# renegade-fi/mpc-jellyfish

Measured on AMD Instinct MI355X. Metric: msm_g1_scalar_pairs_per_s, higher is better.
Workload: dtype u32 (381-bit Fq as 14 x 29-bit limbs, Montgomery)

## Files before the change

mpc-jellyfish_amd/csrc/ecx.cuh:

```cuda
#pragma once
#include "ec.cuh"
#include "fx.cuh"

namespace mzk {

template <class X>
struct AffineX {
    Fx<X> x, y;
    MZK_HD bool is_inf() const {
        uint32_t a = 0;
#pragma unroll
        for (int i = 0; i < X::XN; i++) a |= x.l[i] | y.l[i];
        return a == 0;
    }
};

template <class X>
struct XYZZX {
    Fx<X> x, y, zz, zzz;
    MZK_HD bool is_inf() const {
        uint32_t a = 0;
#pragma unroll
        for (int i = 0; i < X::XN; i++) a |= zz.l[i];
        return a == 0;
    }
    MZK_HD static XYZZX inf() {
        XYZZX r;
        r.x = Fx<X>::one(); r.y = Fx<X>::one(); r.zz = Fx<X>::zero(); r.zzz = Fx<X>::zero();
        return r;
    }
    MZK_HD static XYZZX from_affine(const AffineX<X>& p) {
        if (p.is_inf()) return inf();
        XYZZX r;
        r.x = p.x; r.y = p.y; r.zz = Fx<X>::one(); r.zzz = Fx<X>::one();
        return r;
    }
};

template <class X>
MZK_HD Fx<X> fx_neg_m(const Fx<X>& y) {
    Fx<X> r;
#pragma unroll
    for (int i = 0; i < X::XN; i++) r.l[i] = X::XSUB2[i] - y.l[i];
    return r;
}

template <class X>
MZK_HD XYZZX<X> xyzzx_dbl_affine(const AffineX<X>& p) {
    XYZZX<X> r;
    const Fx<X> u = fx_norm(fx_add(p.y, p.y));
    const Fx<X> v = fx_sqr(u);
    const Fx<X> w = fx_mul(u, v);
    const Fx<X> s = fx_mul(p.x, v);
    const Fx<X> x2 = fx_sqr(p.x);
    const Fx<X> m = fx_norm(fx_add(fx_add(x2, x2), x2));
    const Fx<X> mm = fx_sqr(m);
    r.x = fx_norm(fx_sub_pad<X>(mm, fx_add(s, s), X::XSUB_2S));
    const Fx<X> d = fx_norm(fx_sub_pad<X>(s, r.x, X::XSUB_XY));
    r.y = fx_norm(fx_sub2(fx_mul(m, d), fx_mul(w, p.y)));
    r.zz = v;
    r.zzz = w;
    return r;
}

template <class X>
MZK_HD XYZZX<X> xyzzx_dbl(const XYZZX<X>& p) {
    if (p.is_inf()) return p;
    XYZZX<X> r;
    const Fx<X> u = fx_norm(fx_add(p.y, p.y));
    const Fx<X> v = fx_sqr(u);
    const Fx<X> w = fx_mul(u, v);
    const Fx<X> s = fx_mul(p.x, v);
    const Fx<X> x2 = fx_sqr(p.x);
    const Fx<X> m = fx_norm(fx_add(fx_add(x2, x2), x2));
    const Fx<X> mm = fx_sqr(m);
    r.x = fx_norm(fx_sub_pad<X>(mm, fx_add(s, s), X::XSUB_2S));
    const Fx<X> d = fx_norm(fx_sub_pad<X>(s, r.x, X::XSUB_XY));
    r.y = fx_norm(fx_sub2(fx_mul(m, d), fx_mul(w, p.y)));
    r.zz = fx_mul(v, p.zz);
    r.zzz = fx_mul(w, p.zzz);
    return r;
}

template <class X>
MZK_HD XYZZX<X> xyzzx_madd(const XYZZX<X>& p, const AffineX<X>& q, bool negate) {
    if (q.is_inf()) return p;
    const Fx<X> qy = negate ? fx_neg_m(q.y) : q.y;
    if (p.is_inf()) {
        XYZZX<X> r;
        r.x = q.x; r.y = fx_norm(qy); r.zz = Fx<X>::one(); r.zzz = Fx<X>::one();
        return r;
    }
    const Fx<X> u2 = fx_mul(q.x, p.zz);
    const Fx<X> s2 = fx_mul(qy, p.zzz);
    const Fx<X> pp_ = fx_norm(fx_sub_pad<X>(u2, p.x, X::XSUB_XY));
    const Fx<X> rr_ = fx_norm(fx_sub_pad<X>(s2, p.y, X::XSUB_XY));
    const Fx<X> pp = fx_sqr(pp_);
    const Fx<X> rr2 = fx_sqr(rr_);
    if (fx_is_zero_m(pp)) {
        if (fx_is_zero_m(rr2)) {
            AffineX<X> qq;
            qq.x = q.x;
            qq.y = fx_norm(qy);
            return xyzzx_dbl_affine(qq);
        }
        return XYZZX<X>::inf();
    }
    XYZZX<X> r;
    const Fx<X> ppp = fx_mul(pp_, pp);
    const Fx<X> qv = fx_mul(p.x, pp);
    r.x = fx_norm(fx_sub_pad<X>(rr2, fx_add(ppp, fx_add(qv, qv)), X::XSUB_PQ));
    const Fx<X> d = fx_norm(fx_sub_pad<X>(qv, r.x, X::XSUB_XY));
    r.y = fx_mul2(rr_, d, p.y, fx_neg_m(ppp));
    r.zz = fx_mul(p.zz, pp);
    r.zzz = fx_mul(p.zzz, ppp);
    return r;
}

template <class X>
MZK_HD XYZZX<X> xyzzx_add(const XYZZX<X>& p, const XYZZX<X>& q) {
    if (q.is_inf()) return p;
    if (p.is_inf()) return q;
    const Fx<X> u1 = fx_mul(p.x, q.zz), u2 = fx_mul(q.x, p.zz);
    const Fx<X> s1 = fx_mul(p.y, q.zzz), s2 = fx_mul(q.y, p.zzz);
    const Fx<X> pp_ = fx_norm(fx_sub2(u2, u1));
    const Fx<X> rr_ = fx_norm(fx_sub2(s2, s1));
    const Fx<X> pp = fx_sqr(pp_);
    const Fx<X> rr2 = fx_sqr(rr_);
    if (fx_is_zero_m(pp)) {
        if (fx_is_zero_m(rr2)) return xyzzx_dbl(p);
        return XYZZX<X>::inf();
    }
    XYZZX<X> r;
    const Fx<X> ppp = fx_mul(pp_, pp);
    const Fx<X> qv = fx_mul(u1, pp);
    r.x = fx_norm(fx_sub_pad<X>(rr2, fx_add(ppp, fx_add(qv, qv)), X::XSUB_PQ));
    const Fx<X> d = fx_norm(fx_sub_pad<X>(qv, r.x, X::XSUB_XY));
    r.y = fx_mul2(rr_, d, s1, fx_neg_m(ppp));
    r.zz = fx_mul(fx_mul(p.zz, q.zz), pp);
    r.zzz = fx_mul(fx_mul(p.zzz, q.zzz), ppp);
    return r;
}

#if defined(__HIPCC__)
template <int CTRL, class X>
__device__ __forceinline__ Fx<X> fx_quad_perm(const Fx<X>& a) {
    Fx<X> r;
#pragma unroll
    for (int i = 0; i < X::XN; i++) r.l[i] = (uint32_t)__builtin_amdgcn_update_dpp(0, (int)a.l[i], CTRL, 0xF, 0xF, true);
    return r;
}
template <class X>
__device__ __forceinline__ Fx<X> fx_sel(bool c, const Fx<X>& a, const Fx<X>& b) {
    Fx<X> r;
#pragma unroll
    for (int i = 0; i < X::XN; i++) r.l[i] = c ? a.l[i] : b.l[i];
    return r;
}
constexpr int QP_SWAP2 = 0x4E, QP_SWAP1 = 0xB1, QP_L0 = 0x00, QP_L1 = 0x55, QP_L2 = 0xAA, QP_L3 = 0xFF;

template <class X>
__device__ __forceinline__ Fx<X> xyzzx_add_quad(const Fx<X>& ca, const Fx<X>& cb, int role) {
    const bool r0 = role == 0, r1 = role == 1, hi = role >= 2;
    uint32_t za = 0, zb = 0;
#pragma unroll
    for (int i = 0; i < X::XN; i++) { za |= ca.l[i]; zb |= cb.l[i]; }
    int special = (role == 2 && (za == 0 || zb == 0)) ? 1 : 0;
    const Fx<X> p1 = fx_mul(ca, fx_quad_perm<QP_SWAP2>(cb));
    const Fx<X> d = fx_norm(fx_sub2(fx_quad_perm<QP_SWAP2>(p1), p1));
    const Fx<X> p2 = fx_mul(fx_sel(hi, ca, d), fx_sel(hi, cb, d));
    if (r0 && fx_is_zero_m(p2)) special = 1;
    special |= __builtin_amdgcn_update_dpp(0, special, QP_SWAP1, 0xF, 0xF, true);
    special |= __builtin_amdgcn_update_dpp(0, special, QP_SWAP2, 0xF, 0xF, true);
    if (special) {
        XYZZX<X> a, b;
        a.x = fx_quad_perm<QP_L0>(ca); a.y = fx_quad_perm<QP_L1>(ca); a.zz = fx_quad_perm<QP_L2>(ca); a.zzz = fx_quad_perm<QP_L3>(ca);
        b.x = fx_quad_perm<QP_L0>(cb); b.y = fx_quad_perm<QP_L1>(cb); b.zz = fx_quad_perm<QP_L2>(cb); b.zzz = fx_quad_perm<QP_L3>(cb);
        const XYZZX<X> r = xyzzx_add(a, b);
        return fx_sel(hi, fx_sel(role == 2, r.zz, r.zzz), fx_sel(r0, r.x, r.y));
    }
    const Fx<X> pp = fx_quad_perm<QP_L0>(p2);
    const Fx<X> u1 = fx_quad_perm<QP_L0>(p1);
    const Fx<X> p3 = fx_mul(fx_sel(r0, d, fx_sel(r1, u1, p2)), pp);
    const Fx<X> ppp = fx_quad_perm<QP_L0>(p3);
    const Fx<X> x3 = fx_norm(fx_sub_pad<X>(p2, fx_add(ppp, fx_add(p3, p3)), X::XSUB_PQ));
    const Fx<X> qx = fx_norm(fx_sub_pad<X>(p3, x3, X::XSUB_XY));
    const Fx<X> s1 = fx_quad_perm<QP_L1>(p1);
    const Fx<X> p4 = fx_mul(fx_sel(r0, s1, fx_sel(r1, d, p2)), fx_sel(r1, qx, ppp));
    const Fx<X> y3 = fx_norm(fx_sub2(p4, fx_quad_perm<QP_L0>(p4)));
    const Fx<X> x3_0 = fx_quad_perm<QP_L1>(x3);
    return fx_sel(hi, fx_sel(role == 2, p3, p4), fx_sel(r0, x3_0, y3));
}
#endif

template <class X>
MZK_HD XYZZ<Fp<X>> xyzzx_to_boundary(const XYZZX<X>& p) {
    XYZZ<Fp<X>> r;
    if (p.is_inf()) return XYZZ<Fp<X>>::inf();
    r.x = fx_to_boundary<X>(p.x); r.y = fx_to_boundary<X>(p.y);
    r.zz = fx_to_boundary<X>(p.zz); r.zzz = fx_to_boundary<X>(p.zzz);
    return r;
}

}
```

mpc-jellyfish_amd/csrc/ecz.cuh:

```cuda
#pragma once
#include "ecx.cuh"
#include "fz.cuh"

namespace mzk {

template <class Z>
struct AffineZ {
    Fz<Z> x, y;
    MZK_HD bool is_inf() const {
        int32_t a = 0;
#pragma unroll
        for (int i = 0; i < Z::ZN; i++) a |= x.l[i] | y.l[i];
        return a == 0;
    }
};

template <class Z>
struct XYZZZ {
    Fz<Z> x, y, zz, zzz;
    MZK_HD bool is_inf() const { return fz_is_zero(zz); }
    MZK_HD static XYZZZ inf() {
        XYZZZ r;
        r.x = Fz<Z>::one(); r.y = Fz<Z>::one(); r.zz = Fz<Z>::zero(); r.zzz = Fz<Z>::zero();
        return r;
    }
    MZK_HD static XYZZZ from_affine(const AffineZ<Z>& p) {
        if (p.is_inf()) return inf();
        XYZZZ r;
        r.x = p.x; r.y = p.y; r.zz = Fz<Z>::one(); r.zzz = Fz<Z>::one();
        return r;
    }
};

template <class Z>
MZK_HD void ecz_xy3(Fz<Z>& x3, Fz<Z>& y3, const Fz<Z>& a, const Fz<Z>& b_plus_2c, const Fz<Z>& q, const Fz<Z>& r, const Fz<Z>& y, const Fz<Z>& ppp) {
    x3 = fz_norm_wide(fz_sub(a, b_plus_2c));
    const Fz<Z> d = fz_norm(fz_sub(q, x3));
    y3 = fz_mul2(r, d, y, fz_neg(ppp));
}

template <class Z>
MZK_HD XYZZZ<Z> xyzzz_dbl_affine(const AffineZ<Z>& p) {
    XYZZZ<Z> r;
    const Fz<Z> u = fz_norm(fz_add(p.y, p.y));
    const Fz<Z> v = fz_sqr(u);
    const Fz<Z> w = fz_mul(u, v);
    const Fz<Z> s = fz_mul(p.x, v);
    const Fz<Z> x2 = fz_sqr(p.x);
    const Fz<Z> m = fz_norm_wide(fz_add(fz_add(x2, x2), x2));
    const Fz<Z> mm = fz_sqr(m);
    ecz_xy3<Z>(r.x, r.y, mm, fz_add(s, s), s, m, p.y, w);
    r.zz = v;
    r.zzz = w;
    return r;
}

template <class Z>
MZK_HD XYZZZ<Z> xyzzz_dbl(const XYZZZ<Z>& p) {
    if (p.is_inf()) return p;
    XYZZZ<Z> r;
    const Fz<Z> u = fz_norm(fz_add(p.y, p.y));
    const Fz<Z> v = fz_sqr(u);
    const Fz<Z> w = fz_mul(u, v);
    const Fz<Z> s = fz_mul(p.x, v);
    const Fz<Z> x2 = fz_sqr(p.x);
    const Fz<Z> m = fz_norm_wide(fz_add(fz_add(x2, x2), x2));
    const Fz<Z> mm = fz_sqr(m);
    ecz_xy3<Z>(r.x, r.y, mm, fz_add(s, s), s, m, p.y, w);
    r.zz = fz_mul(v, p.zz);
    r.zzz = fz_mul(w, p.zzz);
    return r;
}

template <class Z>
MZK_HD XYZZZ<Z> xyzzz_madd(const XYZZZ<Z>& p, const AffineZ<Z>& q, bool negate) {
    if (q.is_inf()) return p;
    const Fz<Z> qy = negate ? fz_neg(q.y) : q.y;
    if (p.is_inf()) {
        XYZZZ<Z> r;
        r.x = q.x; r.y = qy; r.zz = Fz<Z>::one(); r.zzz = Fz<Z>::one();
        return r;
    }
    const Fz<Z> u2 = fz_mul(q.x, p.zz);
    const Fz<Z> s2 = fz_mul(qy, p.zzz);
    const Fz<Z> pp_ = fz_norm(fz_sub(u2, p.x));
    const Fz<Z> rr_ = fz_norm(fz_sub(s2, p.y));
    const Fz<Z> pp = fz_sqr(pp_);
    const Fz<Z> rr2 = fz_sqr(rr_);
    if (fz_is_zero(pp)) {
        if (fz_is_zero(rr2)) {
            AffineZ<Z> qq;
            qq.x = q.x;
            qq.y = qy;
            return xyzzz_dbl_affine(qq);
        }
        return XYZZZ<Z>::inf();
    }
    XYZZZ<Z> r;
    const Fz<Z> ppp = fz_mul(pp_, pp);
    const Fz<Z> qv = fz_mul(p.x, pp);
    ecz_xy3<Z>(r.x, r.y, rr2, fz_add(ppp, fz_add(qv, qv)), qv, rr_, p.y, ppp);
    r.zz = fz_mul(p.zz, pp);
    r.zzz = fz_mul(p.zzz, ppp);
    return r;
}

template <class Z>
MZK_HD XYZZZ<Z> xyzzz_add(const XYZZZ<Z>& p, const XYZZZ<Z>& q) {
    if (q.is_inf()) return p;
    if (p.is_inf()) return q;
    const Fz<Z> u1 = fz_mul(p.x, q.zz), u2 = fz_mul(q.x, p.zz);
    const Fz<Z> s1 = fz_mul(p.y, q.zzz), s2 = fz_mul(q.y, p.zzz);
    const Fz<Z> pp_ = fz_norm(fz_sub(u2, u1));
    const Fz<Z> rr_ = fz_norm(fz_sub(s2, s1));
    const Fz<Z> pp = fz_sqr(pp_);
    const Fz<Z> rr2 = fz_sqr(rr_);
    if (fz_is_zero(pp)) {
        if (fz_is_zero(rr2)) return xyzzz_dbl(p);
        return XYZZZ<Z>::inf();
    }
    XYZZZ<Z> r;
    const Fz<Z> ppp = fz_mul(pp_, pp);
    const Fz<Z> qv = fz_mul(u1, pp);
    ecz_xy3<Z>(r.x, r.y, rr2, fz_add(ppp, fz_add(qv, qv)), qv, rr_, s1, ppp);
    r.zz = fz_mul(fz_mul(p.zz, q.zz), pp);
    r.zzz = fz_mul(fz_mul(p.zzz, q.zzz), ppp);
    return r;
}

#if defined(__HIPCC__)
template <int CTRL, class Z>
__device__ __forceinline__ Fz<Z> fz_quad_perm(const Fz<Z>& a) {
    Fz<Z> r;
#pragma unroll
    for (int i = 0; i < Z::ZN; i++) {
        r.l[i] = __builtin_amdgcn_update_dpp(0, a.l[i], CTRL, 0xF, 0xF, true);
        asm("" : "+v"(r.l[i]));
    }
    return r;
}
template <class Z>
__device__ __forceinline__ Fz<Z> fz_sel(bool c, const Fz<Z>& a, const Fz<Z>& b) {
    Fz<Z> r;
#pragma unroll
    for (int i = 0; i < Z::ZN; i++) r.l[i] = c ? a.l[i] : b.l[i];
    return r;
}

template <class Z>
__device__ __forceinline__ Fz<Z> xyzzz_add_quad(const Fz<Z>& ca, const Fz<Z>& cb, int role) {
    const bool r0 = role == 0, r1 = role == 1, hi = role >= 2;
    int special = (role == 2 && (fz_is_zero(ca) || fz_is_zero(cb))) ? 1 : 0;
    const Fz<Z> p1 = fz_mul(ca, fz_quad_perm<QP_SWAP2>(cb));
    const Fz<Z> d = fz_norm(fz_sub(fz_quad_perm<QP_SWAP2>(p1), p1));
    const Fz<Z> p2 = fz_mul(fz_sel(hi, ca, d), fz_sel(hi, cb, d));
    if (r0 && fz_is_zero(p2)) special = 1;
    special |= __builtin_amdgcn_update_dpp(0, special, QP_SWAP1, 0xF, 0xF, true);
    special |= __builtin_amdgcn_update_dpp(0, special, QP_SWAP2, 0xF, 0xF, true);
    if (special) {
        XYZZZ<Z> a, b;
        a.x = fz_quad_perm<QP_L0>(ca); a.y = fz_quad_perm<QP_L1>(ca); a.zz = fz_quad_perm<QP_L2>(ca); a.zzz = fz_quad_perm<QP_L3>(ca);
        b.x = fz_quad_perm<QP_L0>(cb); b.y = fz_quad_perm<QP_L1>(cb); b.zz = fz_quad_perm<QP_L2>(cb); b.zzz = fz_quad_perm<QP_L3>(cb);
        const XYZZZ<Z> r = xyzzz_add(a, b);
        return fz_sel(hi, fz_sel(role == 2, r.zz, r.zzz), fz_sel(r0, r.x, r.y));
    }
    const Fz<Z> pp = fz_quad_perm<QP_L0>(p2);
    const Fz<Z> u1 = fz_quad_perm<QP_L0>(p1);
    const Fz<Z> p3 = fz_mul(fz_sel(r0, d, fz_sel(r1, u1, p2)), pp);
    const Fz<Z> ppp = fz_quad_perm<QP_L0>(p3);
    const Fz<Z> x3 = fz_norm_wide(fz_sub(p2, fz_add(ppp, fz_add(p3, p3))));
    const Fz<Z> qx = fz_norm(fz_sub(p3, x3));
    const Fz<Z> s1 = fz_quad_perm<QP_L1>(p1);
    const Fz<Z> p4 = fz_mul(fz_sel(r0, s1, fz_sel(r1, d, p2)), fz_sel(r1, qx, ppp));
    const Fz<Z> y3 = fz_norm(fz_sub(p4, fz_quad_perm<QP_L0>(p4)));
    const Fz<Z> x3_0 = fz_quad_perm<QP_L1>(x3);
    return fz_sel(hi, fz_sel(role == 2, p3, p4), fz_sel(r0, x3_0, y3));
}
#endif

template <class Z>
MZK_HD XYZZ<Fp<Z>> xyzzz_to_boundary(const XYZZZ<Z>& p) {
    XYZZ<Fp<Z>> r;
    if (p.is_inf()) return XYZZ<Fp<Z>>::inf();
    r.x = fz_to_boundary<Z>(p.x); r.y = fz_to_boundary<Z>(p.y);
    r.zz = fz_to_boundary<Z>(p.zz); r.zzz = fz_to_boundary<Z>(p.zzz);
    return r;
}

}
```

mpc-jellyfish_amd/csrc/msm.cuh:

```cuda
#pragma once
#include <hip/hip_runtime.h>

#include "ec.cuh"
#include "ecx.cuh"
#include "ecz.cuh"

namespace mzk {

constexpr int MSM_THREADS = 256;
constexpr int MSM_ACC_THREADS = 128;
constexpr uint32_t MSM_HEAVY_PER_THREAD = 16;
constexpr uint32_t MSM_HEAVY_RUN = MSM_ACC_THREADS * MSM_HEAVY_PER_THREAD;
constexpr uint32_t MSM_HEAVY_FANIN = MSM_ACC_THREADS * 32;
constexpr int MSM_HEAVY_COUNTERS = 6;
__host__ __device__ inline bool msm_is_heavy(uint32_t count, uint32_t cap) { return count > cap + MSM_HEAVY_RUN; }

inline int msm_choose_window(unsigned long long n) {
    int lg = 0;
    while ((1ull << (lg + 1)) <= n) lg++;
    int c = lg - 2;
    if (c < 4) c = 4;
    if (c > 16) c = 16;
    return c;
}
// ... 86 lines not shown
__global__ __launch_bounds__(1024) void msm_scan_kernel(const uint32_t* __restrict__ hist, uint32_t* __restrict__ offs, uint32_t M) {
    __shared__ uint32_t part[1024];
    const int w = blockIdx.x, t = threadIdx.x;
    const uint32_t per = (M + 1023) / 1024;
    const uint32_t lo = t * per, hi = min(M, lo + per);
    uint32_t sum = 0;
    for (uint32_t b = lo; b < hi; b++) sum += hist[(size_t)w * M + b];
    part[t] = sum;
    __syncthreads();
    for (int d = 1; d < 1024; d <<= 1) {
        uint32_t v = t >= d ? part[t - d] : 0;
        __syncthreads();
        part[t] += v;
        __syncthreads();
    }
    uint32_t run = part[t] - sum;
    for (uint32_t b = lo; b < hi; b++) {
        offs[(size_t)w * M + b] = run;
        run += hist[(size_t)w * M + b];
    }
}

constexpr uint32_t MSM_ORDER_SLICE = 8192;
__device__ __forceinline__ uint32_t order_key(uint32_t count) { return 1023u - min(count, 1023u); }

__global__ __launch_bounds__(1024) void msm_order_hist_kernel(const uint32_t* __restrict__ hist, uint32_t M, uint32_t* __restrict__ keycnt) {
    __shared__ uint32_t cnt[1024];
    const uint32_t w = blockIdx.y, t = threadIdx.x;
    const uint32_t lo = blockIdx.x * MSM_ORDER_SLICE, hi = min(M, lo + MSM_ORDER_SLICE);
    cnt[t] = 0;
    __syncthreads();
    for (uint32_t b = lo + t; b < hi; b += 1024) atomicAdd(&cnt[order_key(hist[(size_t)w * M + b])], 1u);
    __syncthreads();
    if (cnt[t]) atomicAdd(&keycnt[(size_t)w * 1024 + t], cnt[t]);
}
__global__ __launch_bounds__(1024) void msm_order_scan_kernel(uint32_t* __restrict__ keycnt, uint32_t global_sets) {
    __shared__ uint32_t part[1024];
    const uint32_t w = blockIdx.x, t = threadIdx.x;
    uint32_t mine = keycnt[(size_t)w * 1024 + t];
    for (uint32_t s = 1; s < global_sets; s++) mine += keycnt[(size_t)s * 1024 + t];
    part[t] = mine;
    __syncthreads();
    for (int d = 1; d < 1024; d <<= 1) {
        uint32_t v = t >= (uint32_t)d ? part[t - d] : 0;
        __syncthreads();
        part[t] += v;
        __syncthreads();
    }
    keycnt[(size_t)w * 1024 + t] = part[t] - mine;
}
__global__ __launch_bounds__(1024) void msm_order_scatter_kernel(const uint32_t* __restrict__ hist, uint32_t M, uint32_t* __restrict__ keycur,
                                                                 uint32_t* __restrict__ order, bool global) {
    __shared__ uint32_t cnt[1024];
    const uint32_t w = blockIdx.y, t = threadIdx.x;
    const uint32_t row = global ? 0u : w;
    const uint32_t lo = blockIdx.x * MSM_ORDER_SLICE, hi = min(M, lo + MSM_ORDER_SLICE);
    cnt[t] = 0;
    __syncthreads();
    for (uint32_t b = lo + t; b < hi; b += 1024) atomicAdd(&cnt[order_key(hist[(size_t)w * M + b])], 1u);
    __syncthreads();
    const uint32_t mine = cnt[t];
    __syncthreads();
    cnt[t] = mine ? atomicAdd(&keycur[(size_t)row * 1024 + t], mine) : 0u;
    __syncthreads();
    for (uint32_t b = lo + t; b < hi; b += 1024) {
        const uint32_t pos = atomicAdd(&cnt[order_key(hist[(size_t)w * M + b])], 1u);
        order[(size_t)row * M + pos] = w * M + b;
    }
}

struct LongDesc;
struct HeavyRun;
__device__ __forceinline__ void msm_long_register(uint32_t w, uint32_t b, uint32_t c, uint32_t offs_t, int n_win, uint32_t cap, uint32_t desc_cap,
                                                  LongDesc* __restrict__ desc, uint32_t* __restrict__ desc_count, uint32_t run_cap,
                                                  uint32_t h1_cap, HeavyRun* __restrict__ heavy_runs);
__global__ __launch_bounds__(1024) void msm_order_place_kernel(const uint32_t* __restrict__ hist, const uint32_t* __restrict__ offs, uint32_t M,
                                                               const uint32_t* __restrict__ keycnt, uint32_t* __restrict__ keycur, uint32_t* __restrict__ order,
                                                               int n_win, uint32_t cap, uint32_t desc_cap, LongDesc* __restrict__ desc,
                                                               uint32_t* __restrict__ desc_count, uint32_t run_cap, uint32_t h1_cap, HeavyRun* __restrict__ heavy_runs,
                                                               bool global) {
    __shared__ uint32_t cnt[1024];
    __shared__ uint32_t part[1024];
    const uint32_t w = blockIdx.y, t = threadIdx.x;
    const uint32_t row = global ? 0u : w;
    const uint32_t lo = blockIdx.x * MSM_ORDER_SLICE, hi = min(M, lo + MSM_ORDER_SLICE);
    uint32_t total = 0;
    if (global) for (uint32_t s = 0; s < gridDim.y; s++) total += keycnt[(size_t)s * 1024 + t];
    else total = keycnt[(size_t)w * 1024 + t];
    part[t] = total;
    cnt[t] = 0;
    __syncthreads();
    for (int d = 1; d < 1024; d <<= 1) {
        uint32_t v = t >= (uint32_t)d ? part[t - d] : 0;
        __syncthreads();
        part[t] += v;
        __syncthreads();
    }
    const uint32_t key_start = part[t] - total;
    for (uint32_t b = lo + t; b < hi; b += 1024) atomicAdd(&cnt[order_key(hist[(size_t)w * M + b])], 1u);
    __syncthreads();
    const uint32_t mine = cnt[t];
    __syncthreads();
    cnt[t] = mine ? key_start + atomicAdd(&keycur[(size_t)row * 1024 + t], mine) : 0u;
    __syncthreads();
    for (uint32_t b = lo + t; b < hi; b += 1024) {
        const uint32_t c = hist[(size_t)w * M + b];
        const uint32_t pos = atomicAdd(&cnt[order_key(c)], 1u);
        order[(size_t)row * M + pos] = w * M + b;
        if (desc_count && c > cap) msm_long_register(w, b, c, offs[(size_t)w * M + b], n_win, cap, desc_cap, desc, desc_count, run_cap, h1_cap, heavy_runs);
    }
}

template <class FQ>
__device__ __forceinline__ Affine<Fp<FQ>> load_affine(const uint32_t* __restrict__ bases, unsigned long long idx) {
    Affine<Fp<FQ>> p;
    const uint32_t* src = bases + idx * (2 * FQ::N);
    p.x = load_fp<FQ>(src);
    p.y = load_fp<FQ>(src + FQ::N);
    return p;
}
template <class FQ>
__device__ __forceinline__ XYZZ<Fp<FQ>> load_xyzz(const uint32_t* __restrict__ buf, unsigned long long idx) {
    XYZZ<Fp<FQ>> p;
    const uint32_t* src = buf + idx * (4 * FQ::N);
    p.x = load_fp<FQ>(src);
    p.y = load_fp<FQ>(src + FQ::N);
    p.zz = load_fp<FQ>(src + 2 * FQ::N);
    p.zzz = load_fp<FQ>(src + 3 * FQ::N);
    return p;
}
template <class FQ>
__device__ __forceinline__ void store_xyzz(uint32_t* __restrict__ buf, unsigned long long idx, const XYZZ<Fp<FQ>>& p) {
    uint32_t* dst = buf + idx * (4 * FQ::N);
    store_fp<FQ>(dst, p.x);
    store_fp<FQ>(dst + FQ::N, p.y);
    store_fp<FQ>(dst + 2 * FQ::N, p.zz);
    store_fp<FQ>(dst + 3 * FQ::N, p.zzz);
}

template <class FQ>
struct EcFp {
    using Field = FQ;
    using Aff = Affine<Fp<FQ>>;
    using Pt = XYZZ<Fp<FQ>>;
    static constexpr int AFF_WORDS = 2 * FQ::N, PT_WORDS = 4 * FQ::N;
    static __device__ __forceinline__ Aff load_aff(const uint32_t* __restrict__ bases, unsigned long long idx) { return load_affine<FQ>(bases, idx); }
    static __device__ __forceinline__ Pt load_pt(const uint32_t* __restrict__ buf, unsigned long long idx) { return load_xyzz<FQ>(buf, idx); }
    static __device__ __forceinline__ void store_pt(uint32_t* __restrict__ buf, unsigned long long idx, const Pt& p) { store_xyzz<FQ>(buf, idx, p); }
    static __device__ __forceinline__ Pt inf() { return Pt::inf(); }
    static __device__ __forceinline__ Pt madd(const Pt& a, Aff q, bool negate) {
        if (negate) q.y = neg(q.y);
        return xyzz_madd(a, q);
    }
    static __device__ __forceinline__ Pt add(const Pt& a, const Pt& b) { return xyzz_add(a, b); }
    static __device__ __forceinline__ XYZZ<Fp<FQ>> to_boundary(const Pt& p) { return p; }
};

template <class X>
__device__ __forceinline__ void load_words(uint32_t* dst, const uint32_t* __restrict__ src, int n_words) {
    for (int i = 0; i < n_words / 4; i++) {
        const uint4 v = reinterpret_cast<const uint4*>(src)[i];
        dst[4 * i] = v.x; dst[4 * i + 1] = v.y; dst[4 * i + 2] = v.z; dst[4 * i + 3] = v.w;
    }
}

template <class X>
struct EcFx {
    using Field = X;
    using Aff = AffineX<X>;
    using Pt = XYZZX<X>;
    using Fe = Fx<X>;
    static constexpr int LIMBS = X::XN, SLOT_WORDS = X::XN;
    static constexpr int AFF_WORDS = 2 * X::XN, PT_WORDS = 4 * X::XN;
    static_assert((4 * X::XN) % 4 == 0 && (2 * X::XN) % 2 == 0, "points are whole 16-byte / 8-byte words");
    static __device__ __forceinline__ Aff load_aff(const uint32_t* __restrict__ bases, unsigned long long idx) {
        uint32_t w[AFF_WORDS];
        if constexpr (AFF_WORDS % 4 == 0) {
            const uint4* src = reinterpret_cast<const uint4*>(bases + idx * AFF_WORDS);
#pragma unroll
            for (int i = 0; i < AFF_WORDS / 4; i++) {
                const uint4 v = src[i];
                w[4 * i] = v.x; w[4 * i + 1] = v.y; w[4 * i + 2] = v.z; w[4 * i + 3] = v.w;
            }
        } else {
            const uint2* src = reinterpret_cast<const uint2*>(bases + idx * AFF_WORDS);
#pragma unroll
            for (int i = 0; i < AFF_WORDS / 2; i++) {
                const uint2 v = src[i];
                w[2 * i] = v.x; w[2 * i + 1] = v.y;
            }
        }
        Aff p;
#pragma unroll
        for (int i = 0; i < X::XN; i++) { p.x.l[i] = w[i]; p.y.l[i] = w[X::XN + i]; }
        return p;
    }
    static __device__ __forceinline__ Pt load_pt(const uint32_t* __restrict__ buf, unsigned long long idx) {
        uint32_t w[PT_WORDS];
        const uint4* src = reinterpret_cast<const uint4*>(buf + idx * PT_WORDS);
#pragma unroll
        for (int i = 0; i < PT_WORDS / 4; i++) {
            const uint4 v = src[i];
            w[4 * i] = v.x; w[4 * i + 1] = v.y; w[4 * i + 2] = v.z; w[4 * i + 3] = v.w;
        }
        Pt p;
#pragma unroll
        for (int i = 0; i < X::XN; i++) {
            p.x.l[i] = w[i]; p.y.l[i] = w[X::XN + i]; p.zz.l[i] = w[2 * X::XN + i]; p.zzz.l[i] = w[3 * X::XN + i];
        }
        return p;
    }
    static __device__ __forceinline__ void store_pt(uint32_t* __restrict__ buf, unsigned long long idx, const Pt& p) {
        uint32_t w[PT_WORDS];
#pragma unroll
        for (int i = 0; i < X::XN; i++) {
            w[i] = p.x.l[i]; w[X::XN + i] = p.y.l[i]; w[2 * X::XN + i] = p.zz.l[i]; w[3 * X::XN + i] = p.zzz.l[i];
        }
        uint4* dst = reinterpret_cast<uint4*>(buf + idx * PT_WORDS);
#pragma unroll
        for (int i = 0; i < PT_WORDS / 4; i++) dst[i] = make_uint4(w[4 * i], w[4 * i + 1], w[4 * i + 2], w[4 * i + 3]);
    }
    static __device__ __forceinline__ Pt inf() { return Pt::inf(); }
    static __device__ __forceinline__ Pt madd(const Pt& a, const Aff& q, bool negate) { return xyzzx_madd(a, q, negate); }
    static __device__ __forceinline__ Pt add(const Pt& a, const Pt& b) { return xyzzx_add(a, b); }
    static __device__ __forceinline__ XYZZ<Fp<X>> to_boundary(const Pt& p) { return xyzzx_to_boundary(p); }
    static __device__ __forceinline__ Fe add_quad(const Fe& ca, const Fe& cb, int role) { return xyzzx_add_quad<X>(ca, cb, role); }
};

template <class Z>
struct EcFz {
    using Field = Z;
    using Aff = AffineZ<Z>;
    using Pt = XYZZZ<Z>;
    using Fe = Fz<Z>;
    static constexpr int LIMBS = Z::ZN, SLOT_WORDS = Z::ZN + 1;
    static constexpr int AFF_WORDS = 2 * SLOT_WORDS, PT_WORDS = 4 * SLOT_WORDS;
    static_assert(AFF_WORDS % 4 == 0, "points are whole 16-byte words");
    static __device__ __forceinline__ Aff load_aff(const uint32_t* __restrict__ bases, unsigned long long idx) {
        uint32_t w[AFF_WORDS];
        const uint4* src = reinterpret_cast<const uint4*>(bases + idx * AFF_WORDS);
#pragma unroll
        for (int i = 0; i < AFF_WORDS / 4; i++) {
            const uint4 v = src[i];
            w[4 * i] = v.x; w[4 * i + 1] = v.y; w[4 * i + 2] = v.z; w[4 * i + 3] = v.w;
        }
        Aff p;
#pragma unroll
        for (int i = 0; i < LIMBS; i++) { p.x.l[i] = (int32_t)w[i]; p.y.l[i] = (int32_t)w[SLOT_WORDS + i]; }
        return p;
    }
    static __device__ __forceinline__ void store_aff(uint32_t* __restrict__ bases, unsigned long long idx, const Aff& p) {
        uint32_t w[AFF_WORDS];
#pragma unroll
        for (int i = 0; i < LIMBS; i++) { w[i] = (uint32_t)p.x.l[i]; w[SLOT_WORDS + i] = (uint32_t)p.y.l[i]; }
        w[LIMBS] = 0; w[SLOT_WORDS + LIMBS] = 0;
        uint4* dst = reinterpret_cast<uint4*>(bases + idx * AFF_WORDS);
#pragma unroll
        for (int i = 0; i < AFF_WORDS / 4; i++) dst[i] = make_uint4(w[4 * i], w[4 * i + 1], w[4 * i + 2], w[4 * i + 3]);
    }
    static __device__ __forceinline__ Pt load_pt(const uint32_t* __restrict__ buf, unsigned long long idx) {
        uint32_t w[PT_WORDS];
        const uint4* src = reinterpret_cast<const uint4*>(buf + idx * PT_WORDS);
#pragma unroll
        for (int i = 0; i < PT_WORDS / 4; i++) {
            const uint4 v = src[i];
            w[4 * i] = v.x; w[4 * i + 1] = v.y; w[4 * i + 2] = v.z; w[4 * i + 3] = v.w;
        }
        Pt p;
#pragma unroll
        for (int i = 0; i < LIMBS; i++) {
            p.x.l[i] = (int32_t)w[i]; p.y.l[i] = (int32_t)w[SLOT_WORDS + i];
            p.zz.l[i] = (int32_t)w[2 * SLOT_WORDS + i]; p.zzz.l[i] = (int32_t)w[3 * SLOT_WORDS + i];
        }
        return p;
    }
    static __device__ __forceinline__ void store_pt(uint32_t* __restrict__ buf, unsigned long long idx, const Pt& p) {
        uint32_t w[PT_WORDS];
#pragma unroll
        for (int i = 0; i < LIMBS; i++) {
            w[i] = (uint32_t)p.x.l[i]; w[SLOT_WORDS + i] = (uint32_t)p.y.l[i];
            w[2 * SLOT_WORDS + i] = (uint32_t)p.zz.l[i]; w[3 * SLOT_WORDS + i] = (uint32_t)p.zzz.l[i];
        }
#pragma unroll
        for (int k = 0; k < 4; k++) w[k * SLOT_WORDS + LIMBS] = 0;
        uint4* dst = reinterpret_cast<uint4*>(buf + idx * PT_WORDS);
#pragma unroll
        for (int i = 0; i < PT_WORDS / 4; i++) dst[i] = make_uint4(w[4 * i], w[4 * i + 1], w[4 * i + 2], w[4 * i + 3]);
    }
    static __device__ __forceinline__ Pt inf() { return Pt::inf(); }
    static __device__ __forceinline__ Pt madd(const Pt& a, const Aff& q, bool negate) { return xyzzz_madd(a, q, negate); }
    static __device__ __forceinline__ Pt add(const Pt& a, const Pt& b) { return xyzzz_add(a, b); }
    static __device__ __forceinline__ XYZZ<Fp<Z>> to_boundary(const Pt& p) { return xyzzz_to_boundary(p); }
    static __device__ __forceinline__ Fe add_quad(const Fe& ca, const Fe& cb, int role) { return xyzzz_add_quad<Z>(ca, cb, role); }
};

template <class Z>
__global__ __launch_bounds__(MSM_THREADS) void srs_to_internal_z_kernel(const uint32_t* __restrict__ xy, unsigned long long n, uint32_t* __restrict__ out) {
    const unsigned long long i = (unsigned long long)blockIdx.x * MSM_THREADS + threadIdx.x;
    if (i >= n) return;
    const Fp<Z> x = load_fp<Z>(xy + i * 2 * Z::N), y = load_fp<Z>(xy + i * 2 * Z::N + Z::N);
    AffineZ<Z> p;
    p.x = fz_from_boundary<Z>(x);
    p.y = fz_from_boundary<Z>(y);
    EcFz<Z>::store_aff(out, i, p);
}

template <class X>
__global__ __launch_bounds__(MSM_THREADS) void srs_to_internal_kernel(const uint32_t* __restrict__ xy, unsigned long long n, uint32_t* __restrict__ out) {
    const unsigned long long i = (unsigned long long)blockIdx.x * MSM_THREADS + threadIdx.x;
    if (i >= n) return;
    const Fp<X> x = load_fp<X>(xy + i * 2 * X::N), y = load_fp<X>(xy + i * 2 * X::N + X::N);
    const Fx<X> fx = fx_from_boundary<X>(x), fy = fx_from_boundary<X>(y);
    uint32_t* dst = out + i * 2 * X::XN;
#pragma unroll
    for (int k = 0; k < X::XN; k++) { dst[k] = fx.l[k]; dst[X::XN + k] = fy.l[k]; }
}

template <class EC>
__global__ __launch_bounds__(MSM_ACC_THREADS) void msm_accumulate_kernel(const uint32_t* __restrict__ bases, unsigned long long n,
                                                                          const uint32_t* __restrict__ offs, const uint32_t* __restrict__ hist,
                                                                          const uint32_t* __restrict__ sorted, const uint32_t* __restrict__ order,
                                                                          uint32_t M, int n_win, uint32_t cap, uint32_t* __restrict__ long_count,
                                                                          uint32_t* __restrict__ buckets, uint8_t* __restrict__ occ) {
    if (long_count && blockIdx.x == 0)
        for (unsigned i = threadIdx.x; i < (unsigned)n_win * (1 + MSM_HEAVY_COUNTERS); i += MSM_ACC_THREADS) long_count[i] = 0u;
    const unsigned long long t0 = (unsigned long long)blockIdx.x * MSM_ACC_THREADS + threadIdx.x;
    if (t0 >= (unsigned long long)n_win * M) return;
    const uint32_t tb = order[t0];
    const unsigned long long t = tb, w = tb / M;
    const uint32_t start = offs[t];
    const uint32_t h = hist[t];
    const uint32_t cnt = msm_is_heavy(h, cap) ? 0u : min(h, cap);
    const uint32_t* list = sorted + w * n + start;
    typename EC::Pt acc = EC::inf();
    for (uint32_t k = 0; k < cnt; k++) {
        const uint32_t e = list[k];
        acc = EC::madd(acc, EC::load_aff(bases, e & 0x7fffffffu), (e >> 31) != 0);
    }
    const bool empty = acc.is_inf();
    occ[t] = empty ? 0 : 1;
    if (!empty) EC::store_pt(buckets, t, acc);
}

template <class EC, bool ONE_SET>
__global__ __launch_bounds__(MSM_ACC_THREADS) void msm_accumulate_split_kernel(const uint32_t* __restrict__ bases, unsigned long long n,
                                                                                const uint32_t* __restrict__ offs, const uint32_t* __restrict__ hist,
                                                                                const uint32_t* __restrict__ sorted, const uint32_t* __restrict__ order,
                                                                                uint32_t M, int n_win, uint32_t cap, int log_split, uint32_t* __restrict__ long_count,
                                                                                uint32_t* __restrict__ sub, unsigned long long rank0,
                                                                                uint32_t* __restrict__ buckets, uint8_t* __restrict__ occ) {
    if (long_count && blockIdx.x == 0)
        for (unsigned i = threadIdx.x; i < (unsigned)n_win * (1 + MSM_HEAVY_COUNTERS); i += MSM_ACC_THREADS) long_count[i] = 0u;
    const unsigned long long t1 = (unsigned long long)blockIdx.x * MSM_ACC_THREADS + threadIdx.x;
    const bool whole = t1 < rank0;
    const unsigned long long u = whole ? 0ull : t1 - rank0;
    const unsigned long long t0 = whole ? t1 : rank0 + (u >> log_split);
    if (t0 >= (unsigned long long)n_win * M) return;
    const uint32_t S = whole ? 1u : 1u << log_split, part = whole ? 0u : (uint32_t)(u & (S - 1));
    const uint32_t tb = order[t0];
    const unsigned long long t = tb, w = ONE_SET ? 0ull : tb / M;
    const uint32_t start = offs[t];
    const uint32_t h = hist[t];
    const uint32_t cnt = msm_is_heavy(h, cap) ? 0u : min(h, cap);
    const uint32_t* list = sorted + w * n + start;
    typename EC::Pt acc = EC::inf();
    for (uint32_t k = part; k < cnt; k += S) {
        const uint32_t e = list[k];
        acc = EC::madd(acc, EC::load_aff(bases, e & 0x7fffffffu), (e >> 31) != 0);
    }
    if (whole) {
        const bool empty = acc.is_inf();
        occ[t] = empty ? 0 : 1;
        if (!empty) EC::store_pt(buckets, t, acc);
    } else {
        EC::store_pt(sub, u, acc);
    }
}
template <class EC>
__device__ __forceinline__ void pt_lds_put(uint32_t* lds, int slot, const typename EC::Pt& p) {
    constexpr int N = EC::LIMBS;
#pragma unroll
    for (int i = 0; i < N; i++) {
        lds[i * MSM_ACC_THREADS + slot] = p.x.l[i];
        lds[(N + i) * MSM_ACC_THREADS + slot] = p.y.l[i];
        lds[(2 * N + i) * MSM_ACC_THREADS + slot] = p.zz.l[i];
        lds[(3 * N + i) * MSM_ACC_THREADS + slot] = p.zzz.l[i];
    }
}
template <class EC>
__device__ __forceinline__ typename EC::Pt pt_lds_get(const uint32_t* lds, int slot) {
    constexpr int N = EC::LIMBS;
    typename EC::Pt p;
#pragma unroll
    for (int i = 0; i < N; i++) {
        p.x.l[i] = lds[i * MSM_ACC_THREADS + slot];
        p.y.l[i] = lds[(N + i) * MSM_ACC_THREADS + slot];
        p.zz.l[i] = lds[(2 * N + i) * MSM_ACC_THREADS + slot];
        p.zzz.l[i] = lds[(3 * N + i) * MSM_ACC_THREADS + slot];
    }
    return p;
}
template <class EC, bool ONE_SET>
__global__ __launch_bounds__(MSM_ACC_THREADS) void msm_split_combine_kernel(const uint32_t* __restrict__ sub, unsigned long long n_buckets, int log_split,
                                                                             const uint32_t* __restrict__ order, unsigned long long rank0,
                                                                             uint32_t* __restrict__ buckets, uint8_t* __restrict__ occ) {
    __shared__ uint32_t lds[MSM_ACC_THREADS * EC::PT_WORDS];
    const int tid = threadIdx.x;
    const unsigned long long total = n_buckets << log_split;
    const unsigned long long base = (unsigned long long)blockIdx.x * (2 * MSM_ACC_THREADS);
    typename EC::Pt acc = EC::inf();
#pragma unroll 1
    for (int lvl = 0; lvl < log_split; lvl++) {
        const bool mine = tid < (MSM_ACC_THREADS >> lvl) && base + ((unsigned long long)(2 * tid) << lvl) < total;
        typename EC::Pt a = EC::inf(), b = EC::inf();
        if (lvl == 0) {
            if (mine) { a = EC::load_pt(sub, base + 2ull * tid); b = EC::load_pt(sub, base + 2ull * tid + 1); }
        } else {
            __syncthreads();
            if (mine) { a = pt_lds_get<EC>(lds, 2 * tid); b = pt_lds_get<EC>(lds, 2 * tid + 1); }
            __syncthreads();
        }
        if (mine) {
            acc = EC::add(a, b);
            if (lvl == log_split - 1) {
                const unsigned long long t = order[rank0 + (base >> log_split) + tid];
                const bool empty = acc.is_inf();
                occ[t] = empty ? 0 : 1;
                if (!empty) EC::store_pt(buckets, t, acc);
            } else pt_lds_put<EC>(lds, tid, acc);
        }
    }
}

struct LongDesc { uint32_t bucket, start, len, idx_in_run, run_len; };

struct HeavyRun { uint32_t src, n, dest, p1; };
constexpr uint32_t MSM_HEAVY_DEST_PART = 0x80000000u;
constexpr int MSM_HEAVY_JOBS = 8;
struct HeavyJob {
    const uint32_t* bases;
    const uint32_t* sorted;
    unsigned long long n;
    const HeavyRun* runs;
    const uint32_t* count;
    uint32_t *h1, *h2, *h3, *buckets;
    uint8_t* occ;
    uint32_t run_cap, h1_cap, M;
    const LongDesc* desc;
    const uint32_t* desc_count;
    uint32_t* parts;
    uint32_t desc_cap;
};
struct HeavyJobs { HeavyJob j[MSM_HEAVY_JOBS]; };
__device__ __forceinline__ void msm_heavy_push(uint32_t b, uint32_t start, uint32_t rem, uint32_t run_cap, uint32_t h1_cap, uint32_t* __restrict__ cnt,
                                               HeavyRun* __restrict__ runs0, HeavyRun* __restrict__ runsB, HeavyRun* __restrict__ runsC) {
    const uint32_t n1 = (rem + MSM_HEAVY_RUN - 1) / MSM_HEAVY_RUN;
    const uint32_t need = (rem + MSM_HEAVY_PER_THREAD - 1) / MSM_HEAVY_PER_THREAD + n1;
    const uint32_t p1 = atomicAdd(&cnt[5], need);
    if (p1 + need > h1_cap) return;
    const uint32_t r0 = atomicAdd(&cnt[0], n1);
    if (r0 + n1 > run_cap) return;
    constexpr uint32_t PER_RUN = MSM_HEAVY_RUN / MSM_HEAVY_PER_THREAD;
    const uint32_t p2 = atomicAdd(&cnt[3], n1);
    for (uint32_t i = 0; i < n1; i++)
        runs0[r0 + i] = HeavyRun{start + i * MSM_HEAVY_RUN, min(MSM_HEAVY_RUN, rem - i * MSM_HEAVY_RUN), MSM_HEAVY_DEST_PART | (p2 + i), p1 + i * PER_RUN};
    const uint32_t n2 = (n1 + MSM_HEAVY_FANIN - 1) / MSM_HEAVY_FANIN;
    const uint32_t rb = atomicAdd(&cnt[1], n2);
    if (n2 == 1) { runsB[rb] = HeavyRun{p2, n1, b, 0}; return; }
    const uint32_t p3 = atomicAdd(&cnt[4], n2);
    for (uint32_t j = 0; j < n2; j++)
        runsB[rb + j] = HeavyRun{p2 + j * MSM_HEAVY_FANIN, min(MSM_HEAVY_FANIN, n1 - j * MSM_HEAVY_FANIN), MSM_HEAVY_DEST_PART | (p3 + j), 0};
    runsC[atomicAdd(&cnt[2], 1u)] = HeavyRun{p3, n2, b, 0};
}

__device__ __forceinline__ void msm_long_register(uint32_t w, uint32_t b, uint32_t c, uint32_t offs_t, int n_win, uint32_t cap, uint32_t desc_cap,
                                                  LongDesc* __restrict__ desc, uint32_t* __restrict__ desc_count, uint32_t run_cap,
                                                  uint32_t h1_cap, HeavyRun* __restrict__ heavy_runs);

__global__ __launch_bounds__(256) void msm_long_find_kernel(const uint32_t* __restrict__ hist, const uint32_t* __restrict__ offs, uint32_t M, int n_win,
                                                            uint32_t cap, uint32_t desc_cap, LongDesc* __restrict__ desc,
                                                            uint32_t* __restrict__ desc_count, uint32_t run_cap, uint32_t h1_cap, HeavyRun* __restrict__ heavy_runs) {
    const unsigned long long t = (unsigned long long)blockIdx.x * 256 + threadIdx.x;
    if (t >= (unsigned long long)n_win * M) return;
    const uint32_t c = hist[t];
    if (c <= cap) return;
    msm_long_register((uint32_t)(t / M), (uint32_t)(t % M), c, offs[t], n_win, cap, desc_cap, desc, desc_count, run_cap, h1_cap, heavy_runs);
}
__device__ __forceinline__ void msm_long_register(uint32_t w, uint32_t b, uint32_t c, uint32_t offs_t, int n_win, uint32_t cap, uint32_t desc_cap,
                                                  LongDesc* __restrict__ desc, uint32_t* __restrict__ desc_count, uint32_t run_cap,
                                                  uint32_t h1_cap, HeavyRun* __restrict__ heavy_runs) {
    if (msm_is_heavy(c, cap)) {
        HeavyRun* base = heavy_runs + (size_t)w * 3 * run_cap;
        msm_heavy_push(b, offs_t, c, run_cap, h1_cap, desc_count + n_win + (size_t)w * MSM_HEAVY_COUNTERS, base, base + run_cap, base + 2 * (size_t)run_cap);
        return;
    }
    const uint32_t nch = (c - cap + cap - 1) / cap;
    const uint32_t pos = atomicAdd(&desc_count[w], nch);
    if (pos + nch > desc_cap) {
        for (uint32_t i = pos; i < desc_cap; i++) desc[(size_t)w * desc_cap + i] = LongDesc{b, offs_t, 0u, 1u, 0u};
        return;
    }
    for (uint32_t j = 0; j < nch; j++) {
        LongDesc d;
        d.bucket = b;
        d.start = offs_t + cap * (j + 1);
        d.len = min(cap, c - cap * (j + 1));
        d.idx_in_run = j;
        d.run_len = nch;
        desc[(size_t)w * desc_cap + pos + j] = d;
    }
}

template <class EC>
__global__ __launch_bounds__(MSM_ACC_THREADS) void msm_long_chunk_kernel(const uint32_t* __restrict__ bases, unsigned long long n,
                                                                          const uint32_t* __restrict__ sorted, const LongDesc* __restrict__ desc,
                                                                          const uint32_t* __restrict__ desc_count, uint32_t desc_cap,
                                                                          uint32_t* __restrict__ parts) {
    const uint32_t w = blockIdx.y;
    const uint32_t i = blockIdx.x * MSM_ACC_THREADS + threadIdx.x;
    if (i >= min(desc_count[w], desc_cap)) return;
    const LongDesc d = desc[(size_t)w * desc_cap + i];
    const uint32_t* list = sorted + (size_t)w * n + d.start;
// ... 536 lines not shown
```

Before: 347.0 million.

## Add exception-free madd fast path and prefetch next base in bucket accumulation

Replaces the bucket accumulation loop with a helper that prefetches the next scalar index and, for the Z backend, loads the next affine point one iteration ahead. For curve backends that set HAS_REGULAR, the inner loop calls a branch-free madd that only flags exceptional cases (doubling, infinity) and falls back to the full madd when one occurs. The aim is to hide global-memory latency and shorten the divergent special-case logic on the hot path. The costs are extra registers for the prefetched point, which may lower occupancy, and more complex control flow. The X backend (14x29-bit limbs) leaves both flags false, so it only picks up the index prefetch.

```diff
diff --git a/mpc-jellyfish_amd/csrc/ecx.cuh b/mpc-jellyfish_amd/csrc/ecx.cuh
--- a/mpc-jellyfish_amd/csrc/ecx.cuh
+++ b/mpc-jellyfish_amd/csrc/ecx.cuh
@@ -118,6 +118,27 @@
 }
 
 template <class X>
+MZK_HD XYZZX<X> xyzzx_madd_regular(const XYZZX<X>& p, const AffineX<X>& q, bool negate, bool& exc) {
+    const Fx<X> qy = negate ? fx_neg_m(q.y) : q.y;
+    const Fx<X> u2 = fx_mul(q.x, p.zz);
+    const Fx<X> s2 = fx_mul(qy, p.zzz);
+    const Fx<X> pp_ = fx_norm(fx_sub_pad<X>(u2, p.x, X::XSUB_XY));
+    const Fx<X> rr_ = fx_norm(fx_sub_pad<X>(s2, p.y, X::XSUB_XY));
+    const Fx<X> pp = fx_sqr(pp_);
+    const Fx<X> rr2 = fx_sqr(rr_);
+    exc = fx_is_zero_m(pp) || q.is_inf();
+    XYZZX<X> r;
+    const Fx<X> ppp = fx_mul(pp_, pp);
+    const Fx<X> qv = fx_mul(p.x, pp);
+    r.x = fx_norm(fx_sub_pad<X>(rr2, fx_add(ppp, fx_add(qv, qv)), X::XSUB_PQ));
+    const Fx<X> d = fx_norm(fx_sub_pad<X>(qv, r.x, X::XSUB_XY));
+    r.y = fx_mul2(rr_, d, p.y, fx_neg_m(ppp));
+    r.zz = fx_mul(p.zz, pp);
+    r.zzz = fx_mul(p.zzz, ppp);
+    return r;
+}
+
+template <class X>
 MZK_HD XYZZX<X> xyzzx_add(const XYZZX<X>& p, const XYZZX<X>& q) {
     if (q.is_inf()) return p;
     if (p.is_inf()) return q;
diff --git a/mpc-jellyfish_amd/csrc/ecz.cuh b/mpc-jellyfish_amd/csrc/ecz.cuh
--- a/mpc-jellyfish_amd/csrc/ecz.cuh
+++ b/mpc-jellyfish_amd/csrc/ecz.cuh
@@ -96,6 +96,25 @@
         }
         return XYZZZ<Z>::inf();
     }
+    XYZZZ<Z> r;
+    const Fz<Z> ppp = fz_mul(pp_, pp);
+    const Fz<Z> qv = fz_mul(p.x, pp);
+    ecz_xy3<Z>(r.x, r.y, rr2, fz_add(ppp, fz_add(qv, qv)), qv, rr_, p.y, ppp);
+    r.zz = fz_mul(p.zz, pp);
+    r.zzz = fz_mul(p.zzz, ppp);
+    return r;
+}
+
+template <class Z>
+MZK_HD XYZZZ<Z> xyzzz_madd_regular(const XYZZZ<Z>& p, const AffineZ<Z>& q, bool negate, bool& exc) {
+    const Fz<Z> qy = negate ? fz_neg(q.y) : q.y;
+    const Fz<Z> u2 = fz_mul(q.x, p.zz);
+    const Fz<Z> s2 = fz_mul(qy, p.zzz);
+    const Fz<Z> pp_ = fz_norm(fz_sub(u2, p.x));
+    const Fz<Z> rr_ = fz_norm(fz_sub(s2, p.y));
+    const Fz<Z> pp = fz_sqr(pp_);
+    const Fz<Z> rr2 = fz_sqr(rr_);
+    exc = fz_is_zero(pp) || q.is_inf();
     XYZZZ<Z> r;
     const Fz<Z> ppp = fz_mul(pp_, pp);
     const Fz<Z> qv = fz_mul(p.x, pp);
diff --git a/mpc-jellyfish_amd/csrc/msm.cuh b/mpc-jellyfish_amd/csrc/msm.cuh
--- a/mpc-jellyfish_amd/csrc/msm.cuh
+++ b/mpc-jellyfish_amd/csrc/msm.cuh
@@ -262,6 +262,7 @@
         if (negate) q.y = neg(q.y);
         return xyzz_madd(a, q);
     }
+    static constexpr bool HAS_REGULAR = false, POINT_AHEAD = false;
     static __device__ __forceinline__ Pt add(const Pt& a, const Pt& b) { return xyzz_add(a, b); }
     static __device__ __forceinline__ XYZZ<Fp<FQ>> to_boundary(const Pt& p) { return p; }
 };
@@ -332,6 +333,8 @@
     }
     static __device__ __forceinline__ Pt inf() { return Pt::inf(); }
     static __device__ __forceinline__ Pt madd(const Pt& a, const Aff& q, bool negate) { return xyzzx_madd(a, q, negate); }
+    static constexpr bool HAS_REGULAR = false, POINT_AHEAD = false;
+    static __device__ __forceinline__ Pt madd_regular(const Pt& a, const Aff& q, bool negate, bool& exc) { return xyzzx_madd_regular(a, q, negate, exc); }
     static __device__ __forceinline__ Pt add(const Pt& a, const Pt& b) { return xyzzx_add(a, b); }
     static __device__ __forceinline__ XYZZ<Fp<X>> to_boundary(const Pt& p) { return xyzzx_to_boundary(p); }
     static __device__ __forceinline__ Fe add_quad(const Fe& ca, const Fe& cb, int role) { return xyzzx_add_quad<X>(ca, cb, role); }
@@ -399,6 +402,8 @@
     }
     static __device__ __forceinline__ Pt inf() { return Pt::inf(); }
     static __device__ __forceinline__ Pt madd(const Pt& a, const Aff& q, bool negate) { return xyzzz_madd(a, q, negate); }
+    static constexpr bool HAS_REGULAR = true, POINT_AHEAD = true;
+    static __device__ __forceinline__ Pt madd_regular(const Pt& a, const Aff& q, bool negate, bool& exc) { return xyzzz_madd_regular(a, q, negate, exc); }
     static __device__ __forceinline__ Pt add(const Pt& a, const Pt& b) { return xyzzz_add(a, b); }
     static __device__ __forceinline__ XYZZ<Fp<Z>> to_boundary(const Pt& p) { return xyzzz_to_boundary(p); }
     static __device__ __forceinline__ Fe add_quad(const Fe& ca, const Fe& cb, int role) { return xyzzz_add_quad<Z>(ca, cb, role); }
@@ -424,6 +429,46 @@
     uint32_t* dst = out + i * 2 * X::XN;
 #pragma unroll
     for (int k = 0; k < X::XN; k++) { dst[k] = fx.l[k]; dst[X::XN + k] = fy.l[k]; }
+}
+
+template <class EC>
+__device__ __forceinline__ typename EC::Pt accumulate_run(const uint32_t* __restrict__ bases, const uint32_t* __restrict__ list, uint32_t first, uint32_t step,
+                                                          uint32_t cnt) {
+    typename EC::Pt acc = EC::inf();
+    if (first >= cnt) return acc;
+    constexpr bool AHEAD = EC::POINT_AHEAD;
+    uint32_t k = first, e = list[k], e1 = list[k + step < cnt ? k + step : k];
+    typename EC::Aff q, qn;
+    if constexpr (AHEAD) q = EC::load_aff(bases, e & 0x7fffffffu);
+#pragma unroll 1
+    while (k < cnt) {
+        {
+            const uint32_t e2 = list[k + 2 * step < cnt ? k + 2 * step : k];
+            if constexpr (AHEAD) qn = EC::load_aff(bases, e1 & 0x7fffffffu);
+            else q = EC::load_aff(bases, e & 0x7fffffffu);
+            acc = EC::madd(acc, q, (e >> 31) != 0);
+            k += step;
+            e = e1; e1 = e2;
+            if constexpr (AHEAD) q = qn;
+        }
+        if constexpr (EC::HAS_REGULAR) {
+            if (acc.is_inf()) continue;
+#pragma unroll 1
+            while (k < cnt) {
+                const uint32_t e2 = list[k + 2 * step < cnt ? k + 2 * step : k];
+                if constexpr (AHEAD) qn = EC::load_aff(bases, e1 & 0x7fffffffu);
+                else q = EC::load_aff(bases, e & 0x7fffffffu);
+                bool exc;
+                const typename EC::Pt r = EC::madd_regular(acc, q, (e >> 31) != 0, exc);
+                if (exc) break;
+                acc = r;
+                k += step;
+                e = e1; e1 = e2;
+                if constexpr (AHEAD) q = qn;
+            }
+        }
+    }
+    return acc;
 }
 
 template <class EC>
@@ -442,11 +487,7 @@
     const uint32_t h = hist[t];
     const uint32_t cnt = msm_is_heavy(h, cap) ? 0u : min(h, cap);
     const uint32_t* list = sorted + w * n + start;
-    typename EC::Pt acc = EC::inf();
-    for (uint32_t k = 0; k < cnt; k++) {
-        const uint32_t e = list[k];
-        acc = EC::madd(acc, EC::load_aff(bases, e & 0x7fffffffu), (e >> 31) != 0);
-    }
+    const typename EC::Pt acc = accumulate_run<EC>(bases, list, 0u, 1u, cnt);
     const bool empty = acc.is_inf();
     occ[t] = empty ? 0 : 1;
     if (!empty) EC::store_pt(buckets, t, acc);
@@ -473,11 +514,7 @@
     const uint32_t h = hist[t];
     const uint32_t cnt = msm_is_heavy(h, cap) ? 0u : min(h, cap);
     const uint32_t* list = sorted + w * n + start;
-    typename EC::Pt acc = EC::inf();
-    for (uint32_t k = part; k < cnt; k += S) {
-        const uint32_t e = list[k];
-        acc = EC::madd(acc, EC::load_aff(bases, e & 0x7fffffffu), (e >> 31) != 0);
-    }
+    const typename EC::Pt acc = accumulate_run<EC>(bases, list, part, S, cnt);
     if (whole) {
         const bool empty = acc.is_inf();
         occ[t] = empty ? 0 : 1;
```

Result: slower. 342.6 million (-1.3%).
